# arielgabizon/barretenberg

Measured on AMD Instinct MI355X. Metric: BN254 G1 MSM points/sec at n=2^20 (Fr NTT elems/sec in 'ntt'), higher is better.
Workload: dtype u32x9 (256-bit Montgomery, 29-bit limbs)

## Files before the change

barretenberg_amd/csrc/msm.hip:

```cpp
#include <hip/hip_runtime.h>

#include <algorithm>
#include <mutex>
#include <stdint.h>
#include <stdio.h>
#include <stdlib.h>
#include <string.h>
#include <vector>

#include "bbgpu_internal.h"
#include "g1.hpp"
#include "g1_quad.hpp"
#include "host_g1.hpp"

namespace bbgpu {

using Fr = FrP;
#define FRONT_PRIO() __builtin_amdgcn_s_setprio(2)
constexpr int TAIL_PRIO = 3;
constexpr int SCALAR_BITS = 254;
constexpr int MSM_MAX_C = 16;
constexpr int MSM_THREADS = 256;

__device__ __forceinline__ void ld8(const uint32_t* p, uint32_t (&w)[8])
// ... 559 lines not shown
#pragma unroll
        for (int k = 0; k < UB; k++) {
            const uint32_t e = e0 + k * THREADS;
            v[k] = e < end ? tmp[e] : 0u;
        }
        const bool heavy = wave_keys_heavy(e0 < end, (v[0] >> 24) & 0x7f);
#pragma unroll
        for (int k = 0; k < UB; k++)
            if (e0 + k * THREADS < end) (void)lds_inc_dedup(cnt, (v[k] >> 24) & 0x7f, heavy);
    }
    __syncthreads();
    if (t < 128) histB[(((size_t)wl * bins + bin) * parts + part) * 128 + t] = cnt[t];
}
template <int THREADS> __global__ void __launch_bounds__(THREADS) sortB_staged_kernel(const uint32_t* __restrict__ tmp, const uint32_t* __restrict__ binstart,
                                                                                        const uint32_t* __restrict__ bases, uint32_t* __restrict__ sorted,
                                                                                        uint32_t* __restrict__ gstart, uint32_t bins, uint32_t lb, uint32_t nb,
                                                                                        const uint32_t* __restrict__ histB, uint32_t parts_launched)
{
    FRONT_PRIO();
    constexpr int UB = 8;
    constexpr uint32_t TILE = THREADS * UB;
    __shared__ uint32_t cnt[128];
    __shared__ uint32_t cur[128];
    __shared__ uint32_t toff[128];
    __shared__ uint32_t dlt[128];
    __shared__ uint32_t bef[128];
    __shared__ uint32_t buf[TILE];
    const uint32_t bin = blockIdx.x, wl = blockIdx.y, part = blockIdx.z, t = threadIdx.x;
    const uint32_t nlo = 1u << lb;
    const uint32_t bstart = bases[wl] + binstart[(size_t)wl * bins + bin];
    const uint32_t bend = (bin + 1 < bins) ? bases[wl] + binstart[(size_t)wl * bins + bin + 1] : bases[wl + 1];
    const uint32_t len = bend - bstart;
    const uint32_t parts = (parts_launched > 1 && len > SORTB_SPLIT_MIN) ? parts_launched : 1u;
    if (part >= parts) return;
    const uint32_t start = bstart + (uint32_t)(((uint64_t)len * part) / parts), end = bstart + (uint32_t)(((uint64_t)len * (part + 1)) / parts);
    if (t < 128) {
        uint32_t total = 0, before = 0;
        if (parts > 1) {
            const uint32_t* h = histB + (((size_t)wl * bins + bin) * parts) * 128 + t;
            for (uint32_t p = 0; p < parts; p++) {
                const uint32_t c = h[(size_t)p * 128];
                total += c;
                if (p < part) before += c;
            }
        }
        cnt[t] = total;
        bef[t] = before;
    }
    __syncthreads();
    for (uint32_t e0 = start + t; parts == 1 && e0 < end; e0 += TILE) {
        uint32_t v[UB];
#pragma unroll
        for (int k = 0; k < UB; k++) {
            const uint32_t e = e0 + k * THREADS;
            v[k] = e < end ? tmp[e] : 0u;
        }
        const bool heavy = wave_keys_heavy(e0 < end, (v[0] >> 24) & 0x7f);
#pragma unroll
        for (int k = 0; k < UB; k++)
            if (e0 + k * THREADS < end) (void)lds_inc_dedup(cnt, (v[k] >> 24) & 0x7f, heavy);
    }
    __syncthreads();
    if (t < 64) {
        const uint32_t a = cnt[2 * t], b2 = cnt[2 * t + 1], sum = a + b2;
        uint32_t incl = sum;
#pragma unroll
        for (int off = 1; off < 64; off <<= 1) {
            const uint32_t o = __shfl_up(incl, off);
            if ((int)t >= off) incl += o;
        }
        cur[2 * t] = bstart + incl - sum;
        cur[2 * t + 1] = bstart + incl - sum + a;
    }
    __syncthreads();
    if (t < nlo && part == 0) gstart[(size_t)wl * nb + (size_t)bin * nlo + t] = cur[t];
    __syncthreads();
    if (t < 128) cur[t] += bef[t];
    __syncthreads();
    for (uint32_t base = start; base < end; base += TILE) {
        if (t < 128) cnt[t] = 0;
        __syncthreads();
        uint32_t v[UB], rk[UB];
#pragma unroll
        for (int k = 0; k < UB; k++) {
            const uint32_t e = base + k * THREADS + t;
            v[k] = e < end ? tmp[e] : 0u;
        }
        const bool heavy = wave_keys_heavy(base + t < end, (v[0] >> 24) & 0x7f);
#pragma unroll
        for (int k = 0; k < UB; k++) {
            rk[k] = 0u;
            if (base + k * THREADS + t < end) rk[k] = lds_inc_dedup(cnt, (v[k] >> 24) & 0x7f, heavy);
        }
        __syncthreads();
        if (t < 64) {
            const uint32_t a = cnt[2 * t], b2 = cnt[2 * t + 1], sum = a + b2;
            uint32_t incl = sum;
#pragma unroll
            for (int off = 1; off < 64; off <<= 1) {
                const uint32_t o = __shfl_up(incl, off);
                if ((int)t >= off) incl += o;
            }
            const uint32_t x0 = incl - sum, x1 = x0 + a;
            toff[2 * t] = x0;
            toff[2 * t + 1] = x1;
            const uint32_t c0 = cur[2 * t], c1 = cur[2 * t + 1];
            dlt[2 * t] = c0 - x0;
            dlt[2 * t + 1] = c1 - x1;
            cur[2 * t] = c0 + a;
            cur[2 * t + 1] = c1 + b2;
        }
        __syncthreads();
#pragma unroll
        for (int k = 0; k < UB; k++)
            if (base + k * THREADS + t < end) buf[toff[(v[k] >> 24) & 0x7f] + rk[k]] = v[k];
        __syncthreads();
        const uint32_t tile_n = min(TILE, end - base);
        for (uint32_t x = t; x < tile_n; x += THREADS) {
            const uint32_t w = buf[x];
            sorted[dlt[(w >> 24) & 0x7f] + x] = w & 0x80ffffffu;
        }
    }
}

__device__ __forceinline__ void store_raw(uint32_t* dst, const Xyzz& p)
{
#if defined(__HIP_DEVICE_COMPILE__)
    uint32_t v[4 * NL];
#pragma unroll
    for (int i = 0; i < NL; i++) { v[i] = p.x.d[i]; v[NL + i] = p.y.d[i]; v[2 * NL + i] = p.zz.d[i]; v[3 * NL + i] = p.zzz.d[i]; }
#pragma unroll
    for (int i = 0; i < 4 * NL; i += 2)
        asm volatile("global_store_dwordx2 %0, %1, off offset:%2" :: "v"(dst), "v"(((unsigned long long)v[i + 1] << 32) | v[i]), "n"(4 * i) : "memory");
#else
#pragma unroll
    for (int i = 0; i < NL; i++) {
        dst[i] = p.x.d[i];
        dst[NL + i] = p.y.d[i];
        dst[2 * NL + i] = p.zz.d[i];
        dst[3 * NL + i] = p.zzz.d[i];
    }
#endif
}
__device__ __forceinline__ void load_raw(Xyzz& p, const uint32_t* src)
{
#pragma unroll
    for (int i = 0; i < NL; i++) {
        p.x.d[i] = src[i];
        p.y.d[i] = src[NL + i];
        p.zz.d[i] = src[2 * NL + i];
        p.zzz.d[i] = src[3 * NL + i];
    }
}
constexpr int RAW_WORDS = 4 * NL;
constexpr uint32_t HEAVY_WGS = 256;
constexpr uint32_t HEAVY_IDS = 1 + HEAVY_WGS;
static_assert(MSM_THREADS == (int)HEAVY_WGS, "heavy-bucket queue header is cleared / combined by one lane per K4h workgroup");

__global__ void __launch_bounds__(MSM_THREADS) msm_accumulate_kernel(const uint32_t* __restrict__ srs, const uint32_t* __restrict__ sorted,
                                                                   const uint32_t* __restrict__ gstart, uint32_t* __restrict__ partials,
                                                                   uint32_t total_buckets, uint32_t ch, uint32_t prio, uint32_t* __restrict__ heavy_counter)
{
    if (heavy_counter && blockIdx.x == 0) {
        heavy_counter[threadIdx.x] = 0;
        if (threadIdx.x == 0) heavy_counter[MSM_THREADS] = 0;
    }
    if (prio == 1) __builtin_amdgcn_s_setprio(1);
    else if (prio == 2) __builtin_amdgcn_s_setprio(2);
    const uint32_t t = blockIdx.x * blockDim.x + threadIdx.x;
    const uint32_t M = gstart[total_buckets];
    const uint32_t p0 = t * ch;
    if (p0 >= M) return;
    const uint32_t p1 = min(M, p0 + ch);
    uint32_t lo = 0, hi = total_buckets;
    while (hi - lo > 1) {
        const uint32_t mid = (lo + hi) >> 1;
        if (gstart[mid] <= p0) lo = mid; else hi = mid;
    }
    uint32_t b = lo;
    uint32_t next_end = gstart[b + 1];
    Xyzz acc;
    set_infinity(acc);
    uint32_t after_next = gstart[min(b + 2, total_buckets + 1)];
    bool acc_inf = true;
    uint32_t v = sorted[p0];
    uint32_t vn = sorted[p0 + 1 < p1 ? p0 + 1 : p0];
    uint32_t w[16];
    ld16(srs + (size_t)(v & 0x7fffffffu) * 16, w);
    Fe<Fq, 1, 1> px;
    Fe<Fq, 1, 2> py;
    load_affine_m261_signed(px, py, w, (v >> 31) != 0);
    ld16(srs + (size_t)(vn & 0x7fffffffu) * 16, w);
    uint32_t e = p0;
    uint32_t trips = ch;
    do {
        const uint32_t vnn = sorted[min(e + 2, p1 - 1)];
        const bool start = (e == next_end) || acc_inf;
        if (start) {
            if (e == next_end) {
                store_raw(partials + (size_t)(b + t) * RAW_WORDS, acc);
                b++;
                next_end = after_next;
                if (next_end <= e) {
                    if (e >= M) {
                        b = total_buckets;
                    } else {
                        uint32_t l2 = b, h2 = total_buckets;
                        while (h2 - l2 > 1) {
                            const uint32_t mid = (l2 + h2) >> 1;
                            if (gstart[mid] <= e) l2 = mid; else h2 = mid;
                        }
                        b = l2;
                    }
                    next_end = gstart[b + 1];
                }
                after_next = gstart[min(b + 2, total_buckets + 1)];
            }
            acc.x = px;
            acc.y = py;
            acc.zz = fe_one<Fq>();
            acc.zzz = fe_one<Fq>();
            acc_inf = false;
        }
        asm volatile("" ::: "memory");
        if (!start) madd_ip(acc, acc_inf, px, py);
        load_affine_m261_signed(px, py, w, (vn >> 31) != 0);
        ld16(srs + (size_t)(vnn & 0x7fffffffu) * 16, w);
        vn = vnn;
        e++;
    } while (--trips != 0);
    store_raw(partials + (size_t)(b + t) * RAW_WORDS, acc);
}

__device__ __forceinline__ Xyzz shfl_down_xyzz(const Xyzz& p, uint32_t off)
{
    Xyzz r;
#pragma unroll
    for (int i = 0; i < NL; i++) {
        r.x.d[i] = __shfl_down(p.x.d[i], off);
        r.y.d[i] = __shfl_down(p.y.d[i], off);
        r.zz.d[i] = __shfl_down(p.zz.d[i], off);
        r.zzz.d[i] = __shfl_down(p.zzz.d[i], off);
    }
    return r;
}
#define TAIL_OCC __attribute__((amdgpu_waves_per_eu(4, 4)))
constexpr int FOLD_T = 256;
constexpr int FOLD_LDS_WORDS = (FOLD_T / 2) * RAW_WORDS;
__device__ __forceinline__ void wg_tree_sum(Xyzz& acc, uint32_t* sh, uint32_t T, uint32_t t)
{
    constexpr uint32_t STRIDE = FOLD_T / 2;
    for (uint32_t half = T >> 1; half >= 1; half >>= 1) {
        if (t >= half && t < 2 * half) {
#pragma unroll
            for (int i = 0; i < NL; i++) {
                sh[(0 * NL + i) * STRIDE + t - half] = acc.x.d[i];
                sh[(1 * NL + i) * STRIDE + t - half] = acc.y.d[i];
                sh[(2 * NL + i) * STRIDE + t - half] = acc.zz.d[i];
                sh[(3 * NL + i) * STRIDE + t - half] = acc.zzz.d[i];
            }
        }
        __syncthreads();
        if (t < half) {
            Xyzz q, r;
#pragma unroll
            for (int i = 0; i < NL; i++) {
                q.x.d[i] = sh[(0 * NL + i) * STRIDE + t];
                q.y.d[i] = sh[(1 * NL + i) * STRIDE + t];
                q.zz.d[i] = sh[(2 * NL + i) * STRIDE + t];
                q.zzz.d[i] = sh[(3 * NL + i) * STRIDE + t];
            }
            add(r, acc, q);
            acc = r;
        }
        __syncthreads();
    }
}
__global__ void __launch_bounds__(MSM_THREADS) TAIL_OCC msm_merge_kernel(const uint32_t* __restrict__ gstart, const uint32_t* __restrict__ partials,
                                                              uint32_t* __restrict__ buckets, uint32_t* __restrict__ heavy, uint32_t bucket_begin, uint32_t total_buckets,
                                                              uint32_t ch, uint32_t MERGE_LIGHT, uint32_t logG)
{
    __builtin_amdgcn_s_setprio(TAIL_PRIO);
    const uint32_t t = blockIdx.x * blockDim.x + threadIdx.x;
    const uint32_t G = 1u << logG, b = bucket_begin + (t >> logG), j = t & (G - 1);
    if (b >= total_buckets) return;
    const uint32_t s = gstart[b], e = gstart[b + 1];
    Xyzz acc;
    set_infinity(acc);
    if (e > s) {
        const uint32_t t0 = s / ch, t1 = (e - 1) / ch;
        if (t1 - t0 >= MERGE_LIGHT) {
            if (j == 0) heavy[HEAVY_IDS + atomicAdd(&heavy[0], 1u)] = b;
            return;
        }
        for (uint32_t k = t0 + j; k <= t1; k += G) {
            Xyzz q, r;
            load_raw(q, partials + (size_t)(b + k) * RAW_WORDS);
            add(r, acc, q);
            acc = r;
        }
    }
    for (uint32_t off = G >> 1; off >= 1; off >>= 1) {
        const Xyzz o = shfl_down_xyzz(acc, off);
        if (j < off) {
            Xyzz r;
            add(r, acc, o);
            acc = r;
        }
    }
    if (j == 0) {
        uint32_t o[32];
        store_xyzz(o, acc);
        st32(buckets + (size_t)b * 32, o);
    }
}
__global__ void __launch_bounds__(MSM_THREADS) TAIL_OCC msm_merge_heavy_kernel(const uint32_t* __restrict__ gstart, const uint32_t* __restrict__ partials,
                                                                    uint32_t* __restrict__ buckets, uint32_t* __restrict__ heavy, uint32_t ch, uint32_t* __restrict__ hpart)
{
    __builtin_amdgcn_s_setprio(TAIL_PRIO);
    __shared__ uint32_t sh[FOLD_LDS_WORDS];
    __shared__ uint32_t last_flag;
    const uint32_t count = heavy[0];
    const uint32_t K = count ? gridDim.x / count : 0;
    if (K < 2) {
        for (uint32_t item = blockIdx.x; item < count; item += gridDim.x) {
            const uint32_t b = heavy[HEAVY_IDS + item];
            const uint32_t s = gstart[b], e = gstart[b + 1];
            const uint32_t t0 = s / ch, t1 = (e - 1) / ch;
            Xyzz acc;
            set_infinity(acc);
            for (uint32_t t = t0 + threadIdx.x; t <= t1; t += MSM_THREADS) {
                Xyzz q, r;
                load_raw(q, partials + (size_t)(b + t) * RAW_WORDS);
                add(r, acc, q);
                acc = r;
            }
            __syncthreads();
            wg_tree_sum(acc, sh, MSM_THREADS, threadIdx.x);
            if (threadIdx.x == 0) {
                uint32_t o[32];
                store_xyzz(o, acc);
                st32(buckets + (size_t)b * 32, o);
            }
        }
        return;
    }
    const uint32_t item = blockIdx.x / K, sub = blockIdx.x - item * K;
    if (item >= count) return;
    const uint32_t b = heavy[HEAVY_IDS + item];
    const uint32_t s = gstart[b], e = gstart[b + 1];
    const uint32_t t0 = s / ch, t1 = (e - 1) / ch, total = t1 - t0 + 1;
    const uint32_t lo = t0 + (uint32_t)(((uint64_t)total * sub) / K), hi = t0 + (uint32_t)(((uint64_t)total * (sub + 1)) / K);
    Xyzz acc;
    set_infinity(acc);
    for (uint32_t t = lo + threadIdx.x; t < hi; t += MSM_THREADS) {
        Xyzz q, r;
        load_raw(q, partials + (size_t)(b + t) * RAW_WORDS);
        add(r, acc, q);
        acc = r;
    }
    wg_tree_sum(acc, sh, MSM_THREADS, threadIdx.x);
    if (threadIdx.x == 0) {
        store_raw(hpart + (size_t)blockIdx.x * RAW_WORDS, acc);
        __threadfence();
        last_flag = (atomicAdd(&heavy[1 + item], 1u) == K - 1) ? 1u : 0u;
    }
    __syncthreads();
    if (!last_flag) return;
    __threadfence();
    set_infinity(acc);
    if (threadIdx.x < K) load_raw(acc, hpart + (size_t)(item * K + threadIdx.x) * RAW_WORDS);
    __syncthreads();
    wg_tree_sum(acc, sh, MSM_THREADS, threadIdx.x);
    if (threadIdx.x == 0) {
        uint32_t o[32];
        store_xyzz(o, acc);
        st32(buckets + (size_t)b * 32, o);
    }
}

// ... 108 lines not shown
        uint32_t w[8];
        to_canonical(acc, w);
        quad_store8(buckets + (size_t)b * 32 + 8 * l, w);
    }
}

__global__ void __launch_bounds__(QFOLD_T) TAIL_OCC msm_rowcol_quad_kernel(const uint32_t* __restrict__ buckets, uint32_t* __restrict__ R, uint32_t* __restrict__ Cc,
                                                                  uint32_t H, uint32_t L, uint32_t* __restrict__ zero_out, uint32_t zero_words, uint32_t r0, uint32_t rows)
{
    __builtin_amdgcn_s_setprio(TAIL_PRIO);
    __shared__ uint32_t sh[(QFOLD_T / 64) * 4 * NL];
    const uint32_t g = blockIdx.y, t = threadIdx.x, nb = H * L, l = t & 3, quad = t >> 2;
    if (zero_out) {
        const uint32_t gid = (g * gridDim.x + blockIdx.x) * blockDim.x + t, all = gridDim.y * gridDim.x * blockDim.x;
        for (uint32_t i = gid; i < zero_words; i += all) zero_out[i] = 0;
    }
    const bool row = blockIdx.x < rows;
    const uint32_t idx = row ? r0 + blockIdx.x : blockIdx.x - rows, count = row ? L : rows;
    FqN acc = quad_zero();
    bool first = true;
    for (uint32_t e = quad; e < count; e += QFOLD_T / 4) {
        const size_t b = row ? (size_t)idx * L + e : (size_t)(r0 + e) * L + idx;
        const FqN v = quad_load(buckets + ((size_t)g * nb + b) * 32, l);
        acc = first ? v : quad_add(acc, v, l);
        first = false;
    }
    acc = block_quad_sum(acc, sh, t, min(count, (uint32_t)QFOLD_T / 4));
    if (t < 4) {
        uint32_t w[8];
        to_canonical(acc, w);
        quad_store8((row ? R + ((size_t)g * H + idx) * 32 : Cc + ((size_t)g * L + idx) * 32) + 8 * l, w);
    }
}
constexpr uint32_t ROWCOL_SEG = 4;
__global__ void __launch_bounds__(MSM_THREADS) TAIL_OCC msm_rowcol_seg_kernel(const uint32_t* __restrict__ buckets, uint32_t* __restrict__ segs, uint32_t H, uint32_t L,
                                                                                                                uint32_t* __restrict__ zero_out, uint32_t zero_words)
{
    __builtin_amdgcn_s_setprio(TAIL_PRIO);
    const uint32_t g = blockIdx.y, t = blockIdx.x * blockDim.x + threadIdx.x, nb = H * L;
    if (zero_out) {
        const uint32_t gid = g * gridDim.x * blockDim.x + t, all = gridDim.y * gridDim.x * blockDim.x;
        for (uint32_t i = gid; i < zero_words; i += all) zero_out[i] = 0;
    }
    const uint32_t row_lanes = H * (L / ROWCOL_SEG), col_lanes = L * (H / ROWCOL_SEG);
    if (t >= row_lanes + col_lanes) return;
    size_t b, step, out;
    if (t < row_lanes) {
        const uint32_t per = L / ROWCOL_SEG, r = t / per, sidx = t - r * per;
        b = (size_t)r * L + sidx;
        step = per;
        out = t;
    } else {
        const uint32_t u = t - row_lanes, per = H / ROWCOL_SEG, sidx = u / L, c = u - sidx * L;
        b = (size_t)sidx * L + c;
        step = (size_t)per * L;
        out = (size_t)row_lanes + (size_t)c * per + sidx;
    }
    const uint32_t* src = buckets + ((size_t)g * nb + b) * 32;
    Xyzz acc;
    {
        uint32_t w[32];
        ld32(src, w);
        load_xyzz(acc, w);
    }
    for (uint32_t j = 1; j < ROWCOL_SEG; j++) {
        uint32_t w[32];
        ld32(src + j * step * 32, w);
        Xyzz q, r;
        load_xyzz(q, w);
        add(r, acc, q);
        acc = r;
    }
    uint32_t o[32];
    store_xyzz(o, acc);
    st32(segs + ((size_t)g * (row_lanes + col_lanes) + out) * 32, o);
}
__global__ void __launch_bounds__(64) TAIL_OCC msm_segsum_quad_kernel(const uint32_t* __restrict__ segs, uint32_t* __restrict__ R, uint32_t* __restrict__ Cc, uint32_t H, uint32_t L)
{
    __builtin_amdgcn_s_setprio(TAIL_PRIO);
    const uint32_t g = blockIdx.y, t = threadIdx.x, l = t & 3, quad = t >> 2;
    const uint32_t row_lanes = H * (L / ROWCOL_SEG), col_lanes = L * (H / ROWCOL_SEG);
    const bool row = blockIdx.x < H;
    const uint32_t idx = row ? blockIdx.x : blockIdx.x - H, count = row ? L / ROWCOL_SEG : H / ROWCOL_SEG;
    const uint32_t* src = segs + ((size_t)g * (row_lanes + col_lanes) + (row ? (size_t)idx * count : (size_t)row_lanes + (size_t)idx * count)) * 32;
    FqN acc = quad_zero();
    bool first = true;
    for (uint32_t e = quad; e < count; e += 16) {
        const FqN v = quad_load(src + (size_t)e * 32, l);
        acc = first ? v : quad_add(acc, v, l);
        first = false;
    }
    acc = block_quad_sum<64>(acc, nullptr, t, min(count, 16u));
    if (t < 4) {
        uint32_t w[8];
        to_canonical(acc, w);
        quad_store8((row ? R + ((size_t)g * H + idx) * 32 : Cc + ((size_t)g * L + idx) * 32) + 8 * l, w);
    }
}
__global__ void __launch_bounds__(QFOLD_T) TAIL_OCC msm_final_quad_kernel(const uint32_t* __restrict__ R, const uint32_t* __restrict__ Cc, uint32_t* __restrict__ out,
                                                                 uint32_t hbits, uint32_t lbits)
{
    __builtin_amdgcn_s_setprio(TAIL_PRIO);
    __shared__ uint32_t sh[(QFOLD_T / 64) * 4 * NL];
    const uint32_t g = blockIdx.y, t = threadIdx.x, job = blockIdx.x, l = t & 3, quad = t >> 2;
    const uint32_t H = 1u << hbits, L = 1u << lbits;
    const uint32_t* src;
    uint32_t count, slot, k = 0;
    bool sliced = true;
    if (job == 0) { src = R + (size_t)g * H * 32; count = H; slot = 0; sliced = false; }
    else if (job < 1 + hbits) { k = job - 1; src = R + (size_t)g * H * 32; count = H >> 1; slot = 1 + k; }
    else { k = job - 1 - hbits; src = Cc + (size_t)g * L * 32; count = L >> 1; slot = 32 + k; }
    FqN acc = quad_zero();
    bool first = true;
    for (uint32_t e = quad; e < count; e += QFOLD_T / 4) {
        const FqN v = quad_load(src + (size_t)(sliced ? insert_one_bit(e, k) : e) * 32, l);
        acc = first ? v : quad_add(acc, v, l);
        first = false;
    }
    acc = block_quad_sum(acc, sh, t, min(count, (uint32_t)QFOLD_T / 4));
    if (t < 4) {
        uint32_t w[8];
        to_canonical(m261_to_m256<Fq>(acc), w);
        quad_store8(out + ((size_t)g * 64 + slot) * 32 + 8 * l, w);
    }
}

#define HIPCHK(x)                                                                                                      \
    do {                                                                                                               \
        hipError_t e_ = (x);                                                                                           \
        if (e_ != hipSuccess) {                                                                                        \
            set_error("%s:%d %s -> %s", __FILE__, __LINE__, #x, hipGetErrorString(e_));                                \
            return BBGPU_ERR_HIP;                                                                                      \
        }                                                                                                              \
    } while (0)

int msm_choose_c(size_t n)
{
    int lg = 0;
    while (((size_t)1 << lg) < n) lg++;
    int c = lg - 4;
    if (c < 4) c = 4;
    if (c > MSM_MAX_C) c = MSM_MAX_C;
    return c;
}
int msm_num_windows(int c)
{
    return SCALAR_BITS / c + 1;
}

struct MsmPlan {
    uint32_t n, c, W, nb, hbits, lbits, slices, slice_len, sort_lb, sort_bins;
};
constexpr uint32_t ACC_WG_PER_CU = 3;
constexpr uint32_t ACC_LDS_RESERVE = 41 * 1024;
static uint32_t acc_capacity_lanes()
{
    static const uint32_t lanes = [] {
        int dev = 0, cus = 256;
        (void)hipGetDevice(&dev);
        (void)hipDeviceGetAttribute(&cus, hipDeviceAttributeMultiprocessorCount, dev);
        return (uint32_t)cus * ACC_WG_PER_CU * MSM_THREADS;
    }();
    return lanes;
}
constexpr uint32_t MIN_CHUNK = 8;
constexpr uint64_t TINY_ENTRIES = (uint64_t)1 << 16;
constexpr uint32_t TINY_MIN_CHUNK = 4;
static uint32_t min_chunk(uint64_t m) { return m <= TINY_ENTRIES ? TINY_MIN_CHUNK : MIN_CHUNK; }
static uint32_t chunk_len_m(const uint64_t m)
{
    static const double step[3] = { 6.4, 9.2, 13.4 };
    const uint64_t per_k = (uint64_t)acc_capacity_lanes() / ACC_WG_PER_CU;
    uint32_t best = 0;
    double best_cost = 0.0;
    for (uint32_t k = 1; k <= ACC_WG_PER_CU; k++) {
        const uint32_t ch = std::max<uint32_t>(min_chunk(m), (uint32_t)((m + per_k * k - 1) / (per_k * k)));
        const double cost = ch * step[k - 1];
        if (!best || cost < best_cost) { best = ch; best_cost = cost; }
    }
    return best;
}
static uint32_t chunk_len(size_t n, uint32_t nw)
{
    return chunk_len_m((uint64_t)n * nw);
}
static size_t arena_points(const MsmPlan& P, uint32_t nw)
{
    const size_t H = (size_t)1 << P.hbits, L = (size_t)1 << P.lbits;
    return (size_t)nw * (H + L) + 64;
}
static bool rowcol_two_step(const MsmPlan& P)
{
    return P.hbits + P.lbits >= 15;
}
static size_t seg_points(const MsmPlan& P, uint32_t nw)
{
    const size_t H = (size_t)1 << P.hbits, L = (size_t)1 << P.lbits;
    return rowcol_two_step(P) ? (size_t)nw * 2 * (H * L / ROWCOL_SEG) : 0;
}
static MsmPlan make_plan(size_t n, int c)
{
    MsmPlan P;
    P.n = (uint32_t)n;
    P.c = (uint32_t)c;
    P.W = (uint32_t)msm_num_windows(c);
    P.nb = 1u << (c - 1);
    P.lbits = (c - 1) / 2;
    P.hbits = (c - 1) - P.lbits;
    P.slices = std::max<uint32_t>(1, 512 / P.W);
    P.sort_lb = std::min<uint32_t>(SORT_MAX_LB, (uint32_t)c - 1);
    P.sort_bins = P.nb >> P.sort_lb;
    if ((uint64_t)P.slices * 4096 > n) P.slices = std::max<uint32_t>(1, (uint32_t)(n / 4096));
    P.slice_len = (uint32_t)((n + P.slices - 1) / P.slices);
    return P;
}

struct MsmCarve {
    size_t digits, signs, histA, histB, binstart, bintot, tmp_entries, gstart, totals, heavy, sorted, partials, buckets, arena, segs, end;
    size_t chunks_cap, histB_bytes;
};
static MsmCarve carve(const MsmPlan& P, size_t n, size_t nw, size_t ng)
{
    auto al = [](size_t x) { return (x + 255) & ~(size_t)255; };
    MsmCarve L;
    size_t p = 0;
    const size_t wmax = std::max<size_t>(P.W, nw);
    L.digits = p;      p += al(wmax * n * 2);
    L.signs = p;       p += al(wmax * ((n + 63) / 64) * 8);
    L.histA = p;       p += al(nw * P.slices * 1024 * 4);
    L.histB_bytes = (uint64_t)n * nw >= ((uint64_t)1 << 21) ? (size_t)MSM_MAX_JOBS * 1024 * SORTB_MAX_PARTS * 128 * 4 : 0;
    L.histB = p;       p += al(L.histB_bytes);
    L.binstart = p;    p += al(nw * 1024 * 4 + 256);
    L.bintot = p;      p += al(nw * 1024 * 4 + 256);
    L.tmp_entries = p; p += al(nw * n * 4);
    L.gstart = p;      p += al((ng * P.nb + 2) * 4);
    L.totals = p;      p += al(nw * 8 + 512);
    L.heavy = p;       p += al((ng * P.nb + HEAVY_IDS) * 4 + 256 + (size_t)HEAVY_WGS * RAW_WORDS * 4);
    L.sorted = p;      p += al(nw * n * 4);
    L.chunks_cap = (n * nw + min_chunk(n * nw) - 1) / min_chunk(n * nw) + 1;
    L.partials = p;    p += al((ng * P.nb + L.chunks_cap) * RAW_WORDS * 4);
    L.buckets = p;     p += al(ng * P.nb * 128);
    L.arena = p;       p += al(arena_points(P, (uint32_t)ng) * 128);
    L.segs = p;        p += al(seg_points(P, (uint32_t)ng) * 128);
    L.end = p;
    return L;
}
size_t MsmWorkspace::bytes_needed(size_t n, int c, int nw, int ng)
{
    return carve(make_plan(n, c), n, (size_t)nw, (size_t)(ng > 0 ? ng : nw)).end;
}

int MsmWorkspace::ensure(size_t bytes)
{
    if (bytes <= cap) return BBGPU_OK;
    if (base) (void)dev_free(base);
    base = nullptr;
    cap = 0;
    HIPCHK(dev_malloc((void**)&base, bytes));
    cap = bytes;
    return BBGPU_OK;
}
void MsmWorkspace::release()
{
    if (base) (void)dev_free(base);
    if (h_out) (void)hipHostFree(h_out);
    base = nullptr;
    h_out = nullptr;
    cap = 0;
}

int msm_issue_rows(MsmSlot& S, const uint32_t* d_srs, const uint32_t* d_tab, size_t tab_stride, int tab_c, const uint64_t* d_scalars, size_t n,
                   uint64_t row_begin, uint64_t row_end, hipStream_t st, int want_timing)
{
    if (!d_tab || n == 0 || row_end <= row_begin || row_end > (uint64_t)msm_num_windows(tab_c) * n) return BBGPU_ERR_ARG;
    const int wb = (int)(row_begin / n), we = (int)((row_end + n - 1) / n);
    const uint32_t i0 = (uint32_t)(row_begin - (uint64_t)wb * n), i1 = (uint32_t)(row_end - (uint64_t)(we - 1) * n);
    return msm_issue_batch(S, d_srs, d_tab, tab_stride, tab_c, &d_scalars, 1, n, wb, we, st, want_timing, i0, i1);
}

int msm_issue_buckets(MsmSlot& S, const uint32_t* d_srs, const uint32_t* d_tab, size_t tab_stride, int tab_c, const uint64_t* d_scalars, size_t n,
                      uint32_t share, uint32_t share_count, hipStream_t st, int want_timing)
{
    if (!d_tab || n == 0 || share_count == 0 || share >= share_count) return BBGPU_ERR_ARG;
    const MsmPlan P = make_plan(n, tab_c);
    const uint32_t H = 1u << P.hbits;
    if (share_count > H) return BBGPU_ERR_ARG;
    const uint32_t r0 = (uint32_t)((uint64_t)H * share / share_count), r1 = (uint32_t)((uint64_t)H * (share + 1) / share_count);
    return msm_issue_batch(S, d_srs, d_tab, tab_stride, tab_c, &d_scalars, 1, n, 0, (int)P.W, st, want_timing, 0, 0xffffffffu, r0, r1);
}

constexpr int ACC_RING = AccRing::SIZE;
static int acc_ring_record(MsmSlot& S, hipStream_t st)
{
    AccRing* R = S.acc_ring;
    if (!R) {
        S.acc_seq = 0;
        return BBGPU_OK;
    }
    if (R->seq == 0)
        for (int i = 0; i < ACC_RING; i++) HIPCHK(hipEventCreate(&R->end[i]));
    S.acc_seq = ++R->seq;
    HIPCHK(hipEventRecord(R->end[S.acc_seq % ACC_RING], st));
    return BBGPU_OK;
}
void AccRing::release()
{
    if (seq)
// ... 6 lines not shown
int msm_issue_batch(MsmSlot& S, const uint32_t* d_srs, const uint32_t* d_tab, size_t tab_stride, int tab_c, const uint64_t* const* d_scalars_v, int jobs,
                    size_t n, int wb, int we, hipStream_t st, int want_timing, uint32_t row_i0, uint32_t row_i1, uint32_t brow0, uint32_t brow1)
{
    MsmWorkspace& ws = S.ws;
    const bool append = S.append && S.pending && S.npieces > 0;
    S.append = false;
    if (append && (S.jobs != (uint32_t)jobs || S.npieces >= MSM_MAX_PIECES)) {
        set_error("internal: MSM piece %d does not continue the MSM on this slot", S.npieces);
        return BBGPU_ERR_STATE;
    }
    if (!append) {
        S.jobs = (uint32_t)jobs;
        S.n = n;
        S.pending = false;
        S.timed = false;
        S.npieces = 0;
    } else {
        S.n += n;
    }
    MsmPiece& PC = S.piece[S.npieces];
    PC = MsmPiece{};
    PC.hout_group = S.npieces ? S.piece[S.npieces - 1].hout_group + S.piece[S.npieces - 1].nw : 0u;
    if (n == 0) { PC.trivial = true; S.npieces++; S.pending = true; return BBGPU_OK; }
    if (n > ((size_t)1 << 24)) {
        set_error("MSM of %zu points: at most 2^24 points per call", n);
        return BBGPU_ERR_SIZE;
    }
    const bool hint = S.throughput;
    S.throughput = false;
    const bool table = d_tab != nullptr;
    const int c = table ? tab_c : msm_choose_c(n);
    const MsmPlan P = make_plan(n, c);
    if (wb < 0 || we > (int)P.W || wb >= we) return BBGPU_ERR_ARG;
    if (row_i1 > n) row_i1 = (uint32_t)n;
    if ((row_i0 != 0 || row_i1 != n) && (!table || jobs != 1 || row_i0 >= n || (we - wb == 1 && row_i0 >= row_i1))) return BBGPU_ERR_ARG;
    if (jobs < 1 || jobs > MSM_MAX_JOBS || (jobs > 1 && (!table || wb != 0 || we != (int)P.W))) {
        set_error("batched MSM: 1..%d jobs, window tables and the full window range required", MSM_MAX_JOBS);
        return BBGPU_ERR_ARG;
    }
    const uint32_t BH = 1u << P.hbits, BL = 1u << P.lbits;
    if (brow1 > BH) brow1 = BH;
    const bool bshare = brow0 != 0 || brow1 != BH;
    if (bshare && (!table || jobs != 1 || brow0 >= brow1 || wb != 0 || we != (int)P.W || row_i0 != 0 || row_i1 != n)) return BBGPU_ERR_ARG;
    const uint32_t blo = brow0 * BL, bcnt = (brow1 - brow0) * BL;
    const uint32_t nw1 = (uint32_t)(we - wb);
    const uint32_t nw = nw1 * (uint32_t)jobs;
    const uint32_t G = table ? (uint32_t)jobs : nw1;
    const uint32_t wpg = table ? nw1 : 1u;
    uint32_t sort_lb = P.sort_lb, sort_bins = P.sort_bins;
    if (table) {
        uint32_t want_bins = 512;
        while (sort_bins < want_bins && sort_lb > 3) { sort_lb--; sort_bins <<= 1; }
    }
    uint32_t slices = table ? std::max<uint32_t>(1, P.slices * nw1 / 2) : P.slices;
    if (table && jobs == 1) {
        const uint32_t by_cap = (uint32_t)(((uint64_t)nw * P.slices * 1024) / ((uint64_t)G * sort_bins));
        const uint32_t want = std::min<uint32_t>(std::min<uint32_t>(208, (uint32_t)(n / 2048)), by_cap);
        slices = std::max(slices, want);
    }
    const uint32_t slice_len = (uint32_t)((n + slices - 1) / slices);
    const uint32_t idx_stride = table ? (uint32_t)tab_stride : 0u;
    const uint32_t* points = table ? d_tab : d_srs;
    PC.c = P.c; PC.nw = G; PC.wb = table ? 0u : (uint32_t)wb; PC.hbits = P.hbits; PC.lbits = P.lbits;
    if (PC.hout_group + G > MSM_HOUT_GROUPS) {
        set_error("MSM in %d pieces of %u bucket sets: the result array holds %u", S.npieces + 1, G, MSM_HOUT_GROUPS);
        return BBGPU_ERR_SIZE;
    }
    int rc = ws.ensure(MsmWorkspace::bytes_needed(n, c, (int)nw, (int)G));
    if (rc) return rc;
    if (!ws.h_out) HIPCHK(hipHostMalloc((void**)&ws.h_out, (size_t)MSM_HOUT_GROUPS * 64 * 128));
    if (!S.done) HIPCHK(hipEventCreateWithFlags(&S.done, hipEventDisableTiming));

    const MsmCarve LY = carve(P, n, nw, G);
    if (LY.end > ws.cap) {
        set_error("internal: MSM workspace of %zu bytes, layout needs %zu (n=%zu c=%d nw=%u)", ws.cap, LY.end, n, c, nw);
        return BBGPU_ERR_STATE;
    }
    uint8_t* const p = ws.base;
    void* digits = (void*)(p + LY.digits);
    unsigned long long* signs = (unsigned long long*)(p + LY.signs);
    uint32_t* histA = (uint32_t*)(p + LY.histA);
    uint32_t* histB = (uint32_t*)(p + LY.histB);
    uint32_t* binstart = (uint32_t*)(p + LY.binstart);
    uint32_t* bintot = (uint32_t*)(p + LY.bintot);
    uint32_t* tmp_entries = (uint32_t*)(p + LY.tmp_entries);
    uint32_t* gstart = (uint32_t*)(p + LY.gstart);
    uint32_t* totals = (uint32_t*)(p + LY.totals);
    uint32_t* bases = totals + nw;
    uint32_t* heavy = (uint32_t*)(p + LY.heavy);
    uint32_t* sorted = (uint32_t*)(p + LY.sorted);
    uint32_t* partials = (uint32_t*)(p + LY.partials);
    uint32_t* buckets = (uint32_t*)(p + LY.buckets);
    uint32_t* scratch = (uint32_t*)(p + LY.arena);
    if ((uint64_t)G * slices * sort_bins > (uint64_t)nw * P.slices * 1024 || sort_bins > 1024 ||
        (size_t)G * ((size_t)(1u << P.hbits) + (size_t)(1u << P.lbits)) + 64 > arena_points(P, G)) {
        set_error("internal: MSM launch shape exceeds the workspace layout");
        return BBGPU_ERR_STATE;
    }

    hipEvent_t* ev = S.ev;
    const bool tm = want_timing == 1, tm_acc = want_timing != 0;
    S.timed_light = want_timing == 2;
    if (tm_acc) {
        if (!S.ev[0])
            for (int i = 0; i < 8; i++) HIPCHK(hipEventCreate(&S.ev[i]));
        if (tm) HIPCHK(hipEventRecord(ev[0], st));
        S.timed = true;
    }

    if (bshare) {
        HIPCHK(hipMemsetAsync(scratch, 0, (size_t)G * BH * 128, st));
    }
    ScalarSets sets{};
    for (int j = 0; j < jobs; j++) sets.p[j] = (const uint32_t*)d_scalars_v[j];
    const bool wide = c > 16;
    if (wide) msm_digits_kernel<uint16_t><<<dim3((P.n + MSM_THREADS - 1) / MSM_THREADS, jobs), MSM_THREADS, 0, st>>>(sets, (uint16_t*)digits, signs, P.n, make_layout(c, table), P.W, (uint32_t)wb, (uint32_t)we);
    else msm_digits_kernel<int16_t><<<dim3((P.n + MSM_THREADS - 1) / MSM_THREADS, jobs), MSM_THREADS, 0, st>>>(sets, (int16_t*)digits, signs, P.n, make_layout(c, table), P.W, (uint32_t)wb, (uint32_t)we);
    if (tm) HIPCHK(hipEventRecord(ev[1], st));
    if (wide) sortA_hist_kernel<uint16_t><<<dim3(slices, G), SORT_THREADS, 0, st>>>((const uint16_t*)digits, signs, histA, P.n, sort_bins, sort_lb, slices, slice_len, (uint32_t)wb, wpg, row_i0, row_i1, blo, bcnt);
    else sortA_hist_kernel<int16_t><<<dim3(slices, G), SORT_THREADS, 0, st>>>((const int16_t*)digits, signs, histA, P.n, sort_bins, sort_lb, slices, slice_len, (uint32_t)wb, wpg, row_i0, row_i1, blo, bcnt);
    sortA_colscan_kernel<<<dim3((sort_bins + SORT_THREADS / 64 - 1) / (SORT_THREADS / 64), G), SORT_THREADS, 0, st>>>(histA, bintot, sort_bins, slices);
    sortA_scan_kernel<<<G, SORT_THREADS, 0, st>>>(bintot, binstart, totals, sort_bins, G == 1 ? bases : nullptr, gstart + (size_t)G * P.nb);
    if (G > 1) sort_bases_kernel<<<1, 64, 0, st>>>(totals, bases, gstart + (size_t)G * P.nb, G);
    if ((P.n & 7u) == 0) {
        if (wide) sortA_scatter_staged_kernel<uint16_t><<<dim3(slices, G), SORT_THREADS, 0, st>>>((const uint16_t*)digits, signs, histA, binstart, bases, tmp_entries, P.n, sort_bins, sort_lb, slices,
                                                                                  slice_len, (uint32_t)wb, wpg, idx_stride, P.W, row_i0, row_i1, blo, bcnt);
        else sortA_scatter_staged_kernel<int16_t><<<dim3(slices, G), SORT_THREADS, 0, st>>>((const int16_t*)digits, signs, histA, binstart, bases, tmp_entries, P.n, sort_bins, sort_lb, slices,
                                                                            slice_len, (uint32_t)wb, wpg, idx_stride, P.W, row_i0, row_i1, blo, bcnt);
    } else if (wide) sortA_scatter_kernel<uint16_t><<<dim3(slices, G), SORT_THREADS, 0, st>>>((const uint16_t*)digits, signs, histA, binstart, bases, tmp_entries, P.n, sort_bins, sort_lb, slices,
                                                                   slice_len, (uint32_t)wb, wpg, idx_stride, P.W, row_i0, row_i1, blo, bcnt);
    else sortA_scatter_kernel<int16_t><<<dim3(slices, G), SORT_THREADS, 0, st>>>((const int16_t*)digits, signs, histA, binstart, bases, tmp_entries, P.n, sort_bins, sort_lb, slices,
                                                                   slice_len, (uint32_t)wb, wpg, idx_stride, P.W, row_i0, row_i1, blo, bcnt);
    if (table) {
        uint32_t parts = ((uint64_t)n * nw1 >= ((uint64_t)1 << 21) && G <= MSM_MAX_JOBS) ? SORTB_MAX_PARTS : 1u;
        if ((size_t)G * sort_bins * parts * 128 * 4 > LY.histB_bytes) parts = 1;
        if (parts > 1) sortB_count_kernel<SORT_THREADS><<<dim3(sort_bins, G, parts), SORT_THREADS, 0, st>>>(tmp_entries, binstart, bases, histB, sort_bins, parts);
        sortB_staged_kernel<SORT_THREADS><<<dim3(sort_bins, G, parts), SORT_THREADS, 0, st>>>(tmp_entries, binstart, bases, sorted, gstart, sort_bins, sort_lb, P.nb, histB, parts);
    } else sortB_staged_kernel<256><<<dim3(sort_bins, G), 256, 0, st>>>(tmp_entries, binstart, bases, sorted, gstart, sort_bins, sort_lb, P.nb, nullptr, 1u);
    if (tm_acc) HIPCHK(hipEventRecord(ev[2], st));
    const uint32_t total_buckets = G * P.nb;
    const uint64_t m_expected = bshare ? std::max<uint64_t>(1, (uint64_t)n * nw * bcnt / P.nb) : (uint64_t)n * nw;
    const uint32_t merge_buckets = bshare ? bcnt : total_buckets;
    const bool tp = hint && jobs == 1;
    constexpr uint32_t TP_MIN_CHUNK = 20;
    uint32_t ch = bshare ? chunk_len_m(m_expected) : chunk_len(n, nw);
    ch = std::max(ch, min_chunk((uint64_t)n * nw));
    if (tp && ch < TP_MIN_CHUNK)
        ch = std::max(ch, std::min<uint32_t>(TP_MIN_CHUNK, (uint32_t)(m_expected / (acc_capacity_lanes() / ACC_WG_PER_CU))));
    const uint32_t avg_partials = (uint32_t)(m_expected / ((uint64_t)merge_buckets * ch)) + 1;
    uint32_t logG = 0;
    while ((1u << logG) < avg_partials && logG < 6 && ((uint64_t)merge_buckets << (logG + 1)) <= ((uint64_t)1 << 16)) logG++;
    const uint32_t merge_light = std::max(6u, 8u << logG);
    const uint32_t max_chunks = (uint32_t)(((uint64_t)n * nw + ch - 1) / ch);
    msm_accumulate_kernel<<<(max_chunks + MSM_THREADS - 1) / MSM_THREADS, MSM_THREADS, ACC_LDS_RESERVE, st>>>(points, sorted, gstart, partials, total_buckets, ch, 0, heavy);
    if (tm_acc) {
        HIPCHK(hipEventRecord(ev[3], st));
        if (int rc = acc_ring_record(S, st)) return rc;
    } else {
        S.acc_seq = 0;
    }
    if ((uint64_t)n * nw <= ((uint64_t)1 << 21)) {
        uint32_t logQ = 0;
        while ((2u << logQ) < avg_partials && logQ < 4 && ((uint64_t)merge_buckets << (logQ + 3)) <= ((uint64_t)1 << 17)) logQ++;
        msm_merge_quad_kernel<<<(uint32_t)((((uint64_t)merge_buckets << (logQ + 2)) + MSM_THREADS - 1) / MSM_THREADS), MSM_THREADS, 0, st>>>(gstart, partials, buckets, heavy, blo, blo + merge_buckets, ch,
                                                                                                                                  std::max(32u, 8u << logQ), logQ);
    } else msm_merge_kernel<<<(uint32_t)((((uint64_t)merge_buckets << logG) + MSM_THREADS - 1) / MSM_THREADS), MSM_THREADS, 0, st>>>(gstart, partials, buckets, heavy,
                                                                                                                     blo, blo + merge_buckets, ch, merge_light, logG);
    msm_merge_heavy_kernel<<<HEAVY_WGS, MSM_THREADS, 0, st>>>(gstart, partials, buckets, heavy, ch, heavy + (((size_t)G * P.nb + HEAVY_IDS + 63) & ~(size_t)63));
    if (tm) HIPCHK(hipEventRecord(ev[4], st));

    const uint32_t H = 1u << P.hbits, L = 1u << P.lbits;
    {
        uint32_t* Rr = scratch;
        uint32_t* Cc = scratch + (size_t)G * H * 32;
        uint32_t* const dest = (uint32_t*)ws.h_out + (size_t)PC.hout_group * 64 * 32;
        const uint32_t zero_words = G * 64 * 32;
        if (!bshare && rowcol_two_step(P) && (tp || jobs > 1)) {
            uint32_t* segs = (uint32_t*)(p + LY.segs);
            const uint32_t seg_lanes = 2 * (H * L / ROWCOL_SEG);
            msm_rowcol_seg_kernel<<<dim3((seg_lanes + MSM_THREADS - 1) / MSM_THREADS, G), MSM_THREADS, 0, st>>>(buckets, segs, H, L, dest, zero_words);
            msm_segsum_quad_kernel<<<dim3(H + L, G), 64, 0, st>>>(segs, Rr, Cc, H, L);
        } else msm_rowcol_quad_kernel<<<dim3((bshare ? brow1 - brow0 : H) + L, G), QFOLD_T, 0, st>>>(buckets, Rr, Cc, H, L, dest, zero_words, bshare ? brow0 : 0u,
                                                                                                  bshare ? brow1 - brow0 : H);
        if (tm) HIPCHK(hipEventRecord(ev[5], st));
        msm_final_quad_kernel<<<dim3(1 + P.hbits + P.lbits, G), QFOLD_T, 0, st>>>(Rr, Cc, dest, P.hbits, P.lbits);
        if (tm) HIPCHK(hipEventRecord(ev[6], st));
    }
    HIPCHK(hipEventRecord(S.done, st));
    HIPCHK(launch_check());
    S.npieces++;
    S.pending = true;
    return BBGPU_OK;
}

static host::Xyzz group_sum(const MsmSlot& S, const MsmPiece& PC, uint32_t w)
{
    auto pt = [&](uint32_t slot) {
        host::Xyzz q;
        memcpy(&q, (const uint8_t*)S.ws.h_out + ((size_t)(PC.hout_group + w) * 64 + slot) * 128, 128);
        return q;
    };
    host::Xyzz rs = host::g1_infinity();
    for (int k = (int)PC.hbits - 1; k >= 0; --k) rs = host::g1_add(host::g1_dbl(rs), pt(1 + k));
    for (uint32_t k = 0; k < PC.lbits; k++) rs = host::g1_dbl(rs);
    host::Xyzz cs = host::g1_infinity();
    for (int k = (int)PC.lbits - 1; k >= 0; --k) cs = host::g1_add(host::g1_dbl(cs), pt(32 + k));
    return host::g1_add(host::g1_add(rs, cs), pt(0));
}
static int finish_timing(MsmSlot& S, MsmTiming* timing)
{
    if (S.timed && timing) {
        float ms;
        timing->count = 0;
        if (S.timed_light) {
            for (int i = 0; i < 7; i++) timing->ms[timing->count++] = 0.0f;
            HIPCHK(hipEventElapsedTime(&ms, S.ev[2], S.ev[3]));
            timing->ms[3] = ms;
        } else {
            HIPCHK(hipEventElapsedTime(&ms, S.ev[0], S.ev[6]));
            timing->ms[timing->count++] = ms;
            for (int i = 0; i < 6; i++) {
                HIPCHK(hipEventElapsedTime(&ms, S.ev[i], S.ev[i + 1]));
                timing->ms[timing->count++] = ms;
            }
        }
        float exec = timing->ms[3];
        const AccRing* R = S.acc_ring;
        if (R && S.acc_seq > 1 && R->seq - (S.acc_seq - 1) < (uint64_t)ACC_RING &&
            hipEventElapsedTime(&ms, R->end[(S.acc_seq - 1) % ACC_RING], R->end[S.acc_seq % ACC_RING]) == hipSuccess && ms > 0.0f && ms < exec)
            exec = ms;
        (void)hipGetLastError();
        timing->ms[timing->count++] = exec;
    }
    return BBGPU_OK;
}
static int msm_finish(MsmSlot& S, host::Xyzz* result, MsmTiming* timing)
{
    *result = host::g1_infinity();
    if (!S.pending) return BBGPU_ERR_STATE;
    if (S.jobs > 1) return BBGPU_ERR_STATE;
    S.pending = false;
    bool waited = false;
    host::Xyzz total = host::g1_infinity();
    for (int pi = 0; pi < S.npieces; pi++) {
        const MsmPiece& PC = S.piece[pi];
        if (PC.trivial) continue;
        if (!waited) HIPCHK(hipEventSynchronize(S.done));
        waited = true;
        host::Xyzz acc = host::g1_infinity();
        for (int w = (int)PC.nw - 1; w >= 0; --w) {
            for (uint32_t k = 0; k < PC.c; k++) acc = host::g1_dbl(acc);
            acc = host::g1_add(acc, group_sum(S, PC, (uint32_t)w));
        }
        for (uint32_t k = 0; k < PC.c * PC.wb; k++) acc = host::g1_dbl(acc);
        total = host::g1_add(total, acc);
    }
    *result = total;
    if (!waited) return BBGPU_OK;
    return finish_timing(S, timing);
}
int msm_finish_batch(MsmSlot& S, host::Xyzz* results, MsmTiming* timing)
{
    if (S.jobs <= 1) return msm_finish(S, results, timing);
    if (!S.pending) return BBGPU_ERR_STATE;
    S.pending = false;
    for (uint32_t j = 0; j < S.jobs; j++) results[j] = host::g1_infinity();
    bool waited = false;
    for (int pi = 0; pi < S.npieces; pi++) {
        const MsmPiece& PC = S.piece[pi];
        if (PC.trivial) continue;
        if (!waited) HIPCHK(hipEventSynchronize(S.done));
        waited = true;
        for (uint32_t j = 0; j < S.jobs; j++) results[j] = host::g1_add(results[j], group_sum(S, PC, j));
    }
    if (!waited) return BBGPU_OK;
    return finish_timing(S, timing);
}

void MsmSlot::release()
{
    ws.release();
    if (done) (void)hipEventDestroy(done);
    done = nullptr;
    for (auto& e : ev) {
        if (e) (void)hipEventDestroy(e);
        e = nullptr;
    }
    if (stream) (void)hipStreamDestroy(stream);
    stream = nullptr;
    pending = false;
    npieces = 0;
    helper = -1;
    is_helper = append = false;
}

int srs_upload(const uint64_t* host_table, size_t n, uint32_t** d_srs_out, hipStream_t st, size_t stride_bytes)
{
    DevBuf tab, srs;
    HIPCHK(dev_malloc(&tab.p, n * stride_bytes));
    HIPCHK(dev_malloc(&srs.p, n * 64));
    if (int rc = host_to_device(tab.p, host_table, n * stride_bytes, st)) return rc;
    srs_convert_kernel<<<(uint32_t)((n + 127) / 128), 128, 0, st>>>(tab.as<uint32_t>(), srs.as<uint32_t>(), (uint32_t)n, (uint32_t)(stride_bytes / 4));
    HIPCHK(launch_check());
    HIPCHK(hipStreamSynchronize(st));
    *d_srs_out = srs.release<uint32_t>();
    return BBGPU_OK;
}
// ... 60 lines not shown
```

Measured before the change: 889.7 million.

## Prefetch next point row with inline-asm loads and drop accumulate LDS reservation

Replaces the plain 16-word point load in the MSM bucket-accumulate loop with explicit inline-asm global_load_dwordx4 requests issued one iteration ahead. A manual s_waitcnt waits for them just before the point is converted. Compiler barriers keep the loads from being rescheduled, so memory latency should overlap the madd. The 41 KB dynamic LDS reservation on the accumulate launch is also removed, which changes occupancy from the fixed three workgroups per CU it capped. The hand-coded waitcnt assumes a specific count of outstanding vector-memory operations and could be wrong if the compiler interleaves other loads.

Result: faster. 910.5 million, median of 6 (+2.3%).

```diff
diff --git a/barretenberg_amd/csrc/msm.hip b/barretenberg_amd/csrc/msm.hip
--- a/barretenberg_amd/csrc/msm.hip
+++ b/barretenberg_amd/csrc/msm.hip
@@ -735,6 +735,43 @@
         p.zzz.d[i] = src[3 * NL + i];
     }
 }
+typedef uint32_t u32x4 __attribute__((ext_vector_type(4)));
+struct RowRegs { u32x4 q0, q1, q2, q3; };
+__device__ __forceinline__ void row_request(RowRegs& r, const uint32_t* p)
+{
+#if defined(__HIP_DEVICE_COMPILE__)
+    asm volatile("global_load_dwordx4 %0, %4, off\n\t"
+                 "global_load_dwordx4 %1, %4, off offset:16\n\t"
+                 "global_load_dwordx4 %2, %4, off offset:32\n\t"
+                 "global_load_dwordx4 %3, %4, off offset:48"
+                 : "=&v"(r.q0), "=&v"(r.q1), "=&v"(r.q2), "=&v"(r.q3) : "v"(p) : "memory");
+#else
+    const u32x4* q = reinterpret_cast<const u32x4*>(p);
+    r.q0 = q[0]; r.q1 = q[1]; r.q2 = q[2]; r.q3 = q[3];
+#endif
+}
+__device__ __forceinline__ void row_land(RowRegs& r, uint32_t (&w)[16])
+{
+#if defined(__HIP_DEVICE_COMPILE__)
+    __builtin_amdgcn_s_waitcnt(0x0f70);
+    asm volatile("" : "+v"(r.q0), "+v"(r.q1), "+v"(r.q2), "+v"(r.q3));
+#endif
+#pragma unroll
+    for (int i = 0; i < 4; i++) { w[i] = r.q0[i]; w[4 + i] = r.q1[i]; w[8 + i] = r.q2[i]; w[12 + i] = r.q3[i]; }
+}
+__device__ __forceinline__ void value_landed(uint32_t& v)
+{
+#if defined(__HIP_DEVICE_COMPILE__)
+    asm volatile("" : "+v"(v));
+#endif
+}
+__device__ __forceinline__ void operand_done(Fe<Fq, 1, 1>& x, Fe<Fq, 1, 2>& y)
+{
+#if defined(__HIP_DEVICE_COMPILE__)
+    asm volatile("" : "+v"(x.d[0]), "+v"(x.d[1]), "+v"(x.d[2]), "+v"(x.d[3]), "+v"(x.d[4]), "+v"(x.d[5]), "+v"(x.d[6]), "+v"(x.d[7]), "+v"(x.d[8]));
+    asm volatile("" : "+v"(y.d[0]), "+v"(y.d[1]), "+v"(y.d[2]), "+v"(y.d[3]), "+v"(y.d[4]), "+v"(y.d[5]), "+v"(y.d[6]), "+v"(y.d[7]), "+v"(y.d[8]));
+#endif
+}
 constexpr int RAW_WORDS = 4 * NL;
 constexpr uint32_t HEAVY_WGS = 256;
 constexpr uint32_t HEAVY_IDS = 1 + HEAVY_WGS;
@@ -768,12 +805,15 @@
     bool acc_inf = true;
     uint32_t v = sorted[p0];
     uint32_t vn = sorted[p0 + 1 < p1 ? p0 + 1 : p0];
+    RowRegs row;
     uint32_t w[16];
-    ld16(srs + (size_t)(v & 0x7fffffffu) * 16, w);
+    row_request(row, srs + (size_t)(v & 0x7fffffffu) * 16);
     Fe<Fq, 1, 1> px;
     Fe<Fq, 1, 2> py;
+    row_land(row, w);
     load_affine_m261_signed(px, py, w, (v >> 31) != 0);
-    ld16(srs + (size_t)(vn & 0x7fffffffu) * 16, w);
+    operand_done(px, py);
+    row_request(row, srs + (size_t)(vn & 0x7fffffffu) * 16);
     uint32_t e = p0;
     uint32_t trips = ch;
     do {
@@ -796,6 +836,7 @@
                         b = l2;
                     }
                     next_end = gstart[b + 1];
+                    value_landed(next_end);
                 }
                 after_next = gstart[min(b + 2, total_buckets + 1)];
             }
@@ -807,8 +848,10 @@
         }
         asm volatile("" ::: "memory");
         if (!start) madd_ip(acc, acc_inf, px, py);
+        row_land(row, w);
         load_affine_m261_signed(px, py, w, (vn >> 31) != 0);
-        ld16(srs + (size_t)(vnn & 0x7fffffffu) * 16, w);
+        operand_done(px, py);
+        row_request(row, srs + (size_t)(vnn & 0x7fffffffu) * 16);
         vn = vnn;
         e++;
     } while (--trips != 0);
@@ -1223,7 +1266,6 @@
     uint32_t n, c, W, nb, hbits, lbits, slices, slice_len, sort_lb, sort_bins;
 };
 constexpr uint32_t ACC_WG_PER_CU = 3;
-constexpr uint32_t ACC_LDS_RESERVE = 41 * 1024;
 static uint32_t acc_capacity_lanes()
 {
     static const uint32_t lanes = [] {
@@ -1536,7 +1578,7 @@
     while ((1u << logG) < avg_partials && logG < 6 && ((uint64_t)merge_buckets << (logG + 1)) <= ((uint64_t)1 << 16)) logG++;
     const uint32_t merge_light = std::max(6u, 8u << logG);
     const uint32_t max_chunks = (uint32_t)(((uint64_t)n * nw + ch - 1) / ch);
-    msm_accumulate_kernel<<<(max_chunks + MSM_THREADS - 1) / MSM_THREADS, MSM_THREADS, ACC_LDS_RESERVE, st>>>(points, sorted, gstart, partials, total_buckets, ch, 0, heavy);
+    msm_accumulate_kernel<<<(max_chunks + MSM_THREADS - 1) / MSM_THREADS, MSM_THREADS, 0, st>>>(points, sorted, gstart, partials, total_buckets, ch, 0, heavy);
     if (tm_acc) {
         HIPCHK(hipEventRecord(ev[3], st));
         if (int rc = acc_ring_record(S, st)) return rc;
```
